# ska-sa/dc_sand

Measured on AMD Instinct MI355X. Metric: Gcoeff/s (complex weights) 64ant x 1024beam x 32768chan per GPU, higher is better.
Workload: dtype f32

## Files before the change

### dc_sand_amd/csrc/bf_beamform_i8_kernel.inc

```
template <int FORM, bool FULL, int NW = 4>
__global__ void __launch_bounds__(NW * 64) __attribute__((amdgpu_waves_per_eu(i8_waves_per_eu(FORM, FULL))))
#if BF_I8_WEIGHTED
bf_beamform_i8_w_kernel(const bf_bacc_args a, const bf_weights_args w)
#else
bf_beamform_i8_kernel(const bf_bacc_args a)
#endif
{
    constexpr bool WEIGHTED = BF_I8_WEIGHTED;
#if !BF_I8_WEIGHTED
    const bf_weights_args w{};
#endif
    static_assert(NW == 4 || ((NW == 8 || NW == 16) && FORM == kStaged), "8- and 16-wave workgroups exist for the staged form only");
    static_assert(!WEIGHTED || FORM == kStaged || FORM == kChain, "weights exist for the product's forms only");
    constexpr bool STAGED = FORM == kStaged, SPLIT = FORM == kSplit, CHAIN = FORM == kChain;
    extern __shared__ __attribute__((aligned(16))) char staged[];
    uint32_t bid = BACC_LOGICAL_ID(a);
    const uint32_t wave = __builtin_amdgcn_readfirstlane(threadIdx.x >> 6);
    const uint32_t lane = threadIdx.x & 63u;
    const uint32_t bg = bid % a.n_bgroups;
    bid /= a.n_bgroups;
    const uint32_t tg = bid % a.n_tgroups;
    const uint32_t c = bid / a.n_tgroups;
    const uint32_t nbt_log2 = SPLIT || CHAIN ? 0u : a.nbt_log2;
    const uint32_t nbt = 1u << nbt_log2, tpr = SPLIT ? 1u : (uint32_t)NW >> nbt_log2;
    const uint32_t bt = SPLIT ? 0u : wave & (nbt - 1u), slot = SPLIT ? 0u : wave >> nbt_log2;
    const uint32_t kc = SPLIT || CHAIN ? wave : 0u;
    const uint32_t lm = lane & 15u, lg = lane >> 4;
    const uint32_t bw = (bg * nbt + bt) * 16u;
    const uint32_t tt0 = tg * a.tiles_per_wg;
    const uint32_t tt1 = min(tt0 + a.tiles_per_wg, a.nT16);
    const uint32_t n_blocks = tt1 > tt0 + slot ? (tt1 - tt0 - slot + tpr - 1u) / tpr : 0u;
    const bool idle = bw >= a.B || n_blocks == 0u;
    if (!STAGED && !CHAIN && idle) return;
    const bool has_chunk = !(SPLIT || CHAIN) || 64u * kc < a.A;
    if (STAGED) {
        typedef __attribute__((address_space(3))) void lds_void;
        typedef const __attribute__((address_space(1))) void glb_void;
        const uint32_t bytes = (tt1 - tt0) * a.A * 32u;
        const char *src = reinterpret_cast<const char *>(a.ant) + ((uint64_t)c * a.nT16 + tt0) * a.A * 32u;
        for (uint32_t k = wave; k * 1024u < bytes; k += (uint32_t)NW)
            __builtin_amdgcn_global_load_lds((glb_void *)(src + min(k * 1024u + lane * 16u, bytes - 16u)), (lds_void *)(staged + k * 1024u),
                                             16, 0, 0);
    }

    const uint32_t fw = a.flags[0];
    const uint32_t cls = (fw >> 2) == a.epoch ? (fw & 3u) : DCS_CLASS_FAST_LOW;
    const float fChan = (float)c;
    const float D = a.k.fDenominator, y = a.k.fRcpDenominator;
    const float inv = 1.0f / kFixScale;
    float fac[4] = {inv, inv, inv, inv};
    if constexpr (WEIGHTED && STAGED) {
#pragma unroll
        for (int r = 0; r < 4; r++) fac[r] = w.gs[min(bw + (lane >> 4) + 4u * (uint32_t)r, a.B - 1u)] * inv;
    } else if constexpr (WEIGHTED && CHAIN) {
        fac[0] = w.gs[min(bw + (lane & 15u), a.B - 1u)] * inv;
    }

    const bool shared_w = STAGED && a.share_off != 0u && tpr > 1u && cls != DCS_CLASS_SLOW;
    intx4 wre[3], wim[3];
#pragma unroll
    for (int d = 0; d < 3; d++) wre[d] = wim[d] = intx4{0, 0, 0, 0};
    bool bad_re = false, bad_im = false;
    auto make_coefficients = [&]() {
        const uint32_t beam = bw + 4u * (lm & 3u) + (lm >> 2);
        const bool beam_live = beam < a.B;
        const float *tp = a.terms + 2u * (uint64_t)min(beam, a.B - 1u);
        const float *gp = WEIGHTED ? w.gn + min(beam, a.B - 1u) : nullptr;
        auto planes = [](const uint32_t (&g)[4], uint32_t (&out)[3]) {
            const uint32_t t0 = __builtin_amdgcn_perm(g[1], g[0], 0x05010400u), t1 = __builtin_amdgcn_perm(g[1], g[0], 0x07030602u);
            const uint32_t t2 = __builtin_amdgcn_perm(g[3], g[2], 0x05010400u), t3 = __builtin_amdgcn_perm(g[3], g[2], 0x07030602u);
            out[2] = __builtin_amdgcn_perm(t2, t0, 0x05040100u);
            out[1] = __builtin_amdgcn_perm(t2, t0, 0x07060302u);
            out[0] = __builtin_amdgcn_perm(t3, t1, 0x05040100u);
        };
        auto four = [&](auto gen, auto track, uint32_t q, const floatx2 (&k4)[4], const float (&g4)[4], uint32_t (&nr)[3],
                        uint32_t (&ni)[3]) {
            uint32_t gr[4], gi[4];
#pragma unroll
            for (uint32_t z = 0; z < 4; z++) {
                float re, im;
                gen(k4[z].x, k4[z].y, re, im);
                if constexpr (WEIGHTED) re = g4[z] * re, im = g4[z] * im;
                if (decltype(track)::value) {
                    bad_re |= !(fabsf(re) <= 2.0f);
                    bad_im |= !(fabsf(im) <= 2.0f);
                }
                gr[z] = fixed_word(re), gi[z] = fixed_word(im);
            }
            planes(gr, nr), planes(gi, ni);
            if (!FULL) {
                uint32_t mask = 0;
#pragma unroll
                for (uint32_t z = 0; z < 4; z++) mask |= 64u * kc + 4u * (4u * q + z) + lg < a.A ? 0xffu << (8u * z) : 0u;
#pragma unroll
                for (int d = 0; d < 3; d++) nr[d] &= mask, ni[d] &= mask;
            }
        };
        auto generate = [&](auto gen, auto unrolled) {
            floatx2 kp[16];
            float gw[16];
#pragma unroll
            for (uint32_t z = 0; z < 16; z++) {
                const uint32_t ant = 64u * kc + 4u * z + lg;
                if constexpr (WEIGHTED) {
                    if (decltype(unrolled)::value && z >= 4u) continue;
                    gw[z] = gp[(uint64_t)min(ant, a.A - 1u) * a.B];
                }
                kp[z] = *reinterpret_cast<const floatx2 *>(tp + 2u * (uint64_t)min(ant, a.A - 1u) * a.B);
            }
            if (decltype(unrolled)::value) {
#pragma unroll
                for (uint32_t q = 0; q < 4; q++) {
                    if constexpr (WEIGHTED) {
                        if (q < 3u) {
#pragma unroll
                            for (uint32_t z = 4u * q + 4u; z < 4u * q + 8u; z++) {
                                const uint32_t ant = 64u * kc + 4u * z + lg;
                                gw[z] = gp[(uint64_t)min(ant, a.A - 1u) * a.B];
                                kp[z] = *reinterpret_cast<const floatx2 *>(tp + 2u * (uint64_t)min(ant, a.A - 1u) * a.B);
                            }
                        }
                    }
                    if (shared_w && (q & (tpr - 1u)) != slot) continue;
                    const floatx2 k4[4] = {kp[4 * q], kp[4 * q + 1], kp[4 * q + 2], kp[4 * q + 3]};
                    float g4[4] = {};
                    if constexpr (WEIGHTED) g4[0] = gw[4 * q], g4[1] = gw[4 * q + 1], g4[2] = gw[4 * q + 2], g4[3] = gw[4 * q + 3];
                    uint32_t nr[3], ni[3];
                    four(gen, std::false_type{}, q, k4, g4, nr, ni);
                    if constexpr (CHAIN) {
                        uint32_t *cw = reinterpret_cast<uint32_t *>(staged) + (kc * 6u * 64u + lane) * 4u + q;
#pragma unroll
                        for (int d = 0; d < 3; d++) cw[(uint32_t)d * 256u] = beam_live ? nr[d] : 0u, cw[(3u + (uint32_t)d) * 256u] = beam_live ? ni[d] : 0u;
                    } else {
#pragma unroll
                        for (int d = 0; d < 3; d++) wre[d][q] = (int)nr[d], wim[d][q] = (int)ni[d];
                    }
                }
            } else {
#pragma unroll 1
                for (uint32_t q = 0; q < 4; q++) {
                    const floatx2 k4[4] = {kp[0], kp[1], kp[2], kp[3]};
                    float g4[4] = {};
                    if constexpr (WEIGHTED) {
#pragma unroll
                        for (uint32_t z = 0; z < 4; z++) g4[z] = gp[(uint64_t)min(64u * kc + 4u * (4u * q + z) + lg, a.A - 1u) * a.B];
                    }
                    uint32_t nr[3], ni[3];
                    four(gen, std::true_type{}, q, k4, g4, nr, ni);
                    if constexpr (CHAIN) {
                        uint32_t *cw = reinterpret_cast<uint32_t *>(staged) + (kc * 6u * 64u + lane) * 4u + q;
#pragma unroll
                        for (int d = 0; d < 3; d++) cw[(uint32_t)d * 256u] = beam_live ? nr[d] : 0u, cw[(3u + (uint32_t)d) * 256u] = beam_live ? ni[d] : 0u;
                    } else {
#pragma unroll
                        for (int d = 0; d < 3; d++) {
                            wre[d] = intx4{wre[d][1], wre[d][2], wre[d][3], (int)nr[d]};
                            wim[d] = intx4{wim[d][1], wim[d][2], wim[d][3], (int)ni[d]};
                        }
                    }
#pragma unroll
                    for (uint32_t z = 0; z < 12; z++) kp[z] = kp[z + 4];
                }
            }
            if (!CHAIN && !beam_live) {
#pragma unroll
                for (int d = 0; d < 3; d++) wre[d] = wim[d] = intx4{0, 0, 0, 0};
            }
        };
        if (cls == DCS_CLASS_SLOW) {
            generate([&](float kx, float ky, float &re, float &im) { coeff_slow(kx, ky, fChan, D, re, im); }, std::false_type{});
        } else {
            dispatch_fast(a.k.uDiv3Exact != 0u, cls == DCS_CLASS_FAST_LOW, [&](auto div3, auto lowdeg) {
                generate([&](float kx, float ky, float &re, float &im) {
                    coeff_fast<decltype(div3)::value, decltype(lowdeg)::value>(kx, ky, fChan, D, y, re, im);
                }, std::true_type{});
            });
        }
    };

    const char *ant8 = reinterpret_cast<const char *>(a.ant);
    const uint32_t blk_bytes = a.A * 32u;
    const uint32_t m = lm & 7u;
    const bool second = lm >= 8u;
    const uint32_t last = n_blocks - 1u;
    const uint32_t voff = lg * 32u + m * 4u;
    uint32_t cur[2][16];
    auto arrived = [&](uint32_t (&v)[16]) {
        asm volatile("" : "+v"(v[0]), "+v"(v[1]), "+v"(v[2]), "+v"(v[3]), "+v"(v[4]), "+v"(v[5]), "+v"(v[6]), "+v"(v[7]));
        asm volatile("" : "+v"(v[8]), "+v"(v[9]), "+v"(v[10]), "+v"(v[11]), "+v"(v[12]), "+v"(v[13]), "+v"(v[14]), "+v"(v[15]));
    };
    auto fetch = [&](uint32_t (&dst)[16], uint32_t blk, uint32_t kc) {
        const uint32_t blkA = min(blk, last), blkB = min(blk + 1u, last);
        if (STAGED) {
            const uint32_t at = ((second ? blkB : blkA) * tpr + slot) * blk_bytes + m * 4u;
#pragma unroll
            for (uint32_t p = 0; p < 16; p++)
                dst[p] = *reinterpret_cast<const uint32_t *>(staged + at + (FULL ? lg + 4u * p : min(lg + 4u * p, a.A - 1u)) * 32u);
            return;
        }
        const char *base = ant8 + ((uint64_t)c * a.nT16 + tt0 + blkA * tpr + slot) * blk_bytes;
        const uint32_t hop = second ? (blkB - blkA) * tpr * blk_bytes : 0u;
        if (FULL) {
            const char *b2 = base + 2048u * kc;
            const uint32_t vo = hop + voff;
#pragma unroll
            for (uint32_t p = 0; p < 16; p++) dst[p] = *reinterpret_cast<const uint32_t *>(b2 + vo + 128u * p);
        } else {
#pragma unroll
            for (uint32_t p = 0; p < 16; p++)
                dst[p] = *reinterpret_cast<const uint32_t *>(base + (hop + min(64u * kc + lg + 4u * p, a.A - 1u) * 32u + m * 4u));
        }
    };
    auto transpose = [&](const uint32_t (&v)[16], intx4 (&x)[4]) {
#pragma unroll
        for (int q = 0; q < 4; q++) {
            const uint32_t t0 = __builtin_amdgcn_perm(v[4 * q + 1], v[4 * q], 0x05010400u);
            const uint32_t t1 = __builtin_amdgcn_perm(v[4 * q + 1], v[4 * q], 0x07030602u);
            const uint32_t t2 = __builtin_amdgcn_perm(v[4 * q + 3], v[4 * q + 2], 0x05010400u);
            const uint32_t t3 = __builtin_amdgcn_perm(v[4 * q + 3], v[4 * q + 2], 0x07030602u);
            x[0][q] = (int)__builtin_amdgcn_perm(t2, t0, 0x05040100u);
            x[1][q] = (int)__builtin_amdgcn_perm(t2, t0, 0x07060302u);
            x[2][q] = (int)__builtin_amdgcn_perm(t3, t1, 0x05040100u);
            x[3][q] = (int)__builtin_amdgcn_perm(t3, t1, 0x07060302u);
        }
    };
    const intx4 zero = {0, 0, 0, 0};
    auto contract = [&](const intx4 (&x)[4], floatx4 (&f)[4]) {
#pragma unroll
        for (int v = 0; v < 4; v++) {
            const intx4 s3 = __builtin_amdgcn_mfma_i32_16x16x64_i8((v & 1) ? wim[2] : wre[2], x[v], zero, 0, 0, 0);
            const intx4 s2 = __builtin_amdgcn_mfma_i32_16x16x64_i8((v & 1) ? wim[1] : wre[1], x[v], zero, 0, 0, 0);
            const intx4 s1 = __builtin_amdgcn_mfma_i32_16x16x64_i8((v & 1) ? wim[0] : wre[0], x[v], zero, 0, 0, 0);
#pragma unroll
            for (int r = 0; r < 4; r++) f[v][r] = fmaf((float)s1[r], 65536.0f, (float)(s2[r] * 256 + s3[r]));
        }
    };
    uint32_t nan_re = 0, nan_im = 0;
    const float fNaN = __builtin_nanf("");
    auto poison = [&](int r, floatx4 &o) {
        if ((nan_re >> (4u * lg + (uint32_t)r)) & 1u) o[0] = fNaN, o[2] = fNaN;
        if ((nan_im >> (4u * lg + (uint32_t)r)) & 1u) o[1] = fNaN, o[3] = fNaN;
    };
    const uint32_t bb = bw + lg;
    const uint32_t out_blk = a.B * 128u;
    char *out8 = reinterpret_cast<char *>(a.beams);
    auto out_of = [&](uint32_t blk, int r) {
        const uint32_t blkA = min(blk, last), blkB = min(blk + 1u, last);
        char *base = out8 + ((uint64_t)c * a.nT16 + tt0 + blkA * tpr + slot) * out_blk;
        return reinterpret_cast<floatx4 *>(base + ((second ? (blkB - blkA) * tpr * out_blk : 0u) + bb * 128u + m * 16u + 512u * r));
    };
    auto store = [&](floatx4 *dst, const floatx4 o) {
#ifdef DCS_PROBES
        if (a.plain_stores) {
            *dst = o;
            return;
        }
#endif
        __builtin_nontemporal_store(o, dst);
    };
    auto finish = [&](auto whole, uint32_t blk, const floatx4 (&f)[4]) {
#pragma unroll
        for (int r = 0; r < 4; r++) {
            const float sc = WEIGHTED ? fac[r] : inv;
            floatx4 o = {f[0][r] * sc, f[1][r] * sc, f[2][r] * sc, f[3][r] * sc};
            if (nan_re | nan_im) poison(r, o);
            if (decltype(whole)::value || bb + 4u * r < a.B) {
                floatx4 *dst = out_of(blk, r);
#ifdef DCS_PROBES
                if (a.probe == 4u) {
                    const uint32_t blkA = min(blk, last), blkB = min(blk + 1u, last);
                    dst = reinterpret_cast<floatx4 *>(out8 + ((uint64_t)c * a.nT16 + tt0 + blkA * tpr + slot) * out_blk +
                                                      ((r >= 2 ? (blkB - blkA) * tpr * out_blk : 0u) + bw * 128u + (r & 1) * 1024u + lane * 16u));
                }
#endif
                store(dst, o);
            }
        }
    };
    floatx4 *part = reinterpret_cast<floatx4 *>(staged);
    const uint32_t n_chunks = (a.A + 63u) / 64u;
    auto park = [&](int h, const floatx4 (&f)[4]) {
#pragma unroll
        for (int r = 0; r < 4; r++) {
            floatx4 o = {f[0][r], f[1][r], f[2][r], f[3][r]};
            if (nan_re | nan_im) poison(r, o);
            part[((h * 4 + r) * 4 + kc) * 64u + lane] = o;
        }
    };
    auto gather = [&](auto whole, int h, uint32_t blk) {
        floatx4 o = part[((h * 4 + wave) * 4 + 0) * 64u + lane];
        for (uint32_t k = 1; k < n_chunks; k++) o = o + part[((h * 4 + wave) * 4 + k) * 64u + lane];
        o = o * inv;
        if (decltype(whole)::value || bb + 4u * wave < a.B) store(out_of(blk, (int)wave), o);
    };
    auto run = [&](auto whole) {
#ifdef DCS_PROBES
        if (!SPLIT && (a.probe == 1u || a.probe == 3u || a.probe == 4u)) {
            floatx4 f[4];
#pragma unroll
            for (int v = 0; v < 4; v++) f[v] = floatx4{(float)wre[0][0], (float)wre[1][1], (float)wim[0][2], (float)wim[2][3]};
            for (uint32_t blk = 0; blk < n_blocks; blk += 2) finish(whole, blk, f);
            return;
        }
        if (FORM == kDirect && a.probe == 2u) {
            for (uint32_t blk = 0; blk < n_blocks; blk += 4) {
                arrived(cur[0]);
                arrived(cur[1]);
#pragma unroll
                for (int h = 0; h < 2; h++) {
                    floatx4 f[4];
#pragma unroll
                    for (int v = 0; v < 4; v++)
                        f[v] = floatx4{(float)cur[h][4 * v], (float)cur[h][4 * v + 1], (float)cur[h][4 * v + 2], (float)cur[h][4 * v + 3]};
                    finish(whole, blk + 2u * h, f);
                }
                __builtin_amdgcn_sched_barrier(0);
                fetch(cur[0], blk + 4u, kc);
                fetch(cur[1], blk + 6u, kc);
            }
            return;
        }
#endif
        if (STAGED) {
            for (uint32_t blk = 0; blk < n_blocks; blk += 2) {
                intx4 x[4];
                floatx4 f[4];
                fetch(cur[0], blk, 0u);
                transpose(cur[0], x);
                contract(x, f);
                finish(whole, blk, f);
            }
        } else {
            for (uint32_t blk = 0; blk < n_blocks; blk += 4) {
                if (has_chunk) {
                    arrived(cur[0]);
                    arrived(cur[1]);
#pragma unroll
                    for (int h = 0; h < 2; h++) {
                        intx4 x[4];
                        floatx4 f[4];
                        transpose(cur[h], x);
                        contract(x, f);
                        if (SPLIT)
                            park(h, f);
                        else
                            finish(whole, blk + 2u * h, f);
                    }
                }
                if (SPLIT) {
                    __syncthreads();
                    gather(whole, 0, blk);
                    gather(whole, 1, blk + 2u);
                    __syncthreads();
                }
                __builtin_amdgcn_sched_barrier(0);
                if (has_chunk) {
                    fetch(cur[0], blk + 4u, kc);
                    fetch(cur[1], blk + 6u, kc);
                }
            }
        }
    };
    if (!STAGED && !CHAIN && has_chunk) fetch(cur[0], 0, kc);
    if (CHAIN && !idle) fetch(cur[0], 0, 0u);
    __builtin_amdgcn_sched_barrier(0);
#ifdef DCS_PROBES
    if (a.probe == 3u || a.probe == 4u) {
#pragma unroll
        for (int d = 0; d < 3; d++) wre[d] = wim[d] = intx4{(int)lane, d, 2, 1};
    } else
#endif
    if ((shared_w || CHAIN ? bw < a.B : !idle) && has_chunk) make_coefficients();
    if (cls == DCS_CLASS_SLOW) {
        const uint64_t br = __builtin_amdgcn_ballot_w64(bad_re), bi = __builtin_amdgcn_ballot_w64(bad_im);
        nan_re = (uint32_t)((br | (br >> 16) | (br >> 32) | (br >> 48)) & 0xffffu);
        nan_im = (uint32_t)((bi | (bi >> 16) | (bi >> 32) | (bi >> 48)) & 0xffffu);
    }
    if constexpr (STAGED) {
        uint32_t *wx = reinterpret_cast<uint32_t *>(staged + a.share_off) + bt * (4u * 6u * 64u) + lane;
        if (shared_w && bw < a.B) {
#pragma unroll
            for (uint32_t q = 0; q < 4; q++)
                if ((q & (tpr - 1u)) == slot) {
#pragma unroll
                    for (int d = 0; d < 3; d++) wx[(q * 6u + d) * 64u] = (uint32_t)wre[d][q], wx[(q * 6u + 3u + d) * 64u] = (uint32_t)wim[d][q];
                }
        }
        __syncthreads();
        if (idle) return;
        if (shared_w) {
#pragma unroll
            for (uint32_t q = 0; q < 4; q++)
                if ((q & (tpr - 1u)) != slot) {
#pragma unroll
                    for (int d = 0; d < 3; d++) wre[d][q] = (int)wx[(q * 6u + d) * 64u], wim[d][q] = (int)wx[(q * 6u + 3u + d) * 64u];
                }
        }
    } else if constexpr (CHAIN) {
        intx4 *coef = reinterpret_cast<intx4 *>(staged);
        uint32_t *nanw = reinterpret_cast<uint32_t *>(staged + 4u * 6u * 64u * 16u);
        if (lane == 0u) nanw[2u * wave] = has_chunk ? nan_re : 0u, nanw[2u * wave + 1u] = has_chunk ? nan_im : 0u;
        float *facw = reinterpret_cast<float *>(nanw + 8);
        if constexpr (WEIGHTED) {
            if (wave == 0u && lane < 16u) facw[lane] = fac[0];
        }
        __syncthreads();
        if (idle) return;
        nan_re = nanw[0] | nanw[2] | nanw[4] | nanw[6];
        nan_im = nanw[1] | nanw[3] | nanw[5] | nanw[7];
        const uint32_t n_chunks = (a.A + 63u) / 64u;
        auto run_chain = [&](auto whole) {
            const uint32_t n_steps = ((n_blocks + 1u) >> 1) * n_chunks;
            intx4 acc[4][3];
            uint32_t s = 0, chunk = 0, blk = 0;
            uint32_t f_s = 1u, f_chunk = 1u % n_chunks, f_blk = 2u * (1u / n_chunks);
            auto step = [&](uint32_t (&now)[16], uint32_t (&ahead)[16]) {
                arrived(now);
                if (f_s < n_steps) fetch(ahead, f_blk, f_chunk);
                f_s++;
                if (++f_chunk == n_chunks) f_chunk = 0u, f_blk += 2u;
                intx4 x[4];
                transpose(now, x);
                if (chunk == 0u) {
#pragma unroll
                    for (int v = 0; v < 4; v++)
#pragma unroll
                        for (int d = 0; d < 3; d++) acc[v][d] = zero;
                }
#pragma unroll
                for (int half = 0; half < 2; half++) {
#pragma unroll
                    for (int d = 0; d < 3; d++) {
                        const intx4 w = coef[(chunk * 6u + 3u * (uint32_t)half + (uint32_t)d) * 64u + lane];
#pragma unroll
                        for (int v = half; v < 4; v += 2) acc[v][d] = __builtin_amdgcn_mfma_i32_16x16x64_i8(w, x[v], acc[v][d], 0, 0, 0);
                    }
                }
                if (chunk + 1u == n_chunks) {
                    float sc_next = WEIGHTED ? facw[lg] : inv;
#pragma unroll
                    for (int r = 0; r < 4; r++) {
                        const float sc = sc_next;
                        if constexpr (WEIGHTED) {
                            if (r < 3) sc_next = facw[4u * (uint32_t)r + 4u + lg];
                        }
                        floatx4 o;
#pragma unroll
                        for (int v = 0; v < 4; v++) o[v] = fmaf((float)acc[v][0][r], 65536.0f, (float)(acc[v][1][r] * 256 + acc[v][2][r])) * sc;
                        if (nan_re | nan_im) poison(r, o);
                        if (decltype(whole)::value || bb + 4u * (uint32_t)r < a.B) store(out_of(blk, r), o);
                        __builtin_amdgcn_sched_barrier(0);
                    }
                    chunk = 0u, blk += 2u;
                } else {
                    chunk++;
                }
                s++;
            };
            while (s < n_steps) {
                step(cur[0], cur[1]);
                if (s < n_steps) step(cur[1], cur[0]);
            }
        };
        if (bw + 16u <= a.B)
            run_chain(std::true_type{});
        else
            run_chain(std::false_type{});
        return;
    } else if (has_chunk) {
        fetch(cur[1], 2, kc);
    }
    if (bw + 16u <= a.B)
        run(std::true_type{});
    else
        run(std::false_type{});
}
```

### dc_sand_amd/csrc/bf_beamform_mfma.hip

```cpp

#include "bf_kernels.h"

#include <hip/hip_runtime.h>

#include <type_traits>

#include "bf_device.h"

namespace {

__device__ __forceinline__ uint32_t xcd_grouped(uint32_t w, uint32_t total, uint32_t G) { return bf_xcd_grouped(w, total, G); }
#ifdef DCS_PROBES
__device__ __forceinline__ uint32_t probe_order(uint32_t order, uint32_t w, uint32_t total, uint32_t G, uint32_t n_sharers)
{
    if (order == 1u) return w;
    if (order >= 16u && order < 24u) return (w + (order - 16u)) % total;
    if (order == 2u) {
        const uint32_t per = total >> 3, rem = total & 7u, x = w & 7u, q = w >> 3;
        return x * per + min(x, rem) + q;
    }
    return xcd_grouped(w, total, order == 3u ? n_sharers : G);
}
#define BACC_LOGICAL_ID(a) probe_order((a).order, blockIdx.x, gridDim.x, (a).xcd_group, (a).n_bgroups)
#else
#define BACC_LOGICAL_ID(a) xcd_grouped(blockIdx.x, gridDim.x, (a).xcd_group)
#endif

constexpr uint32_t kKC = 64;

template <int NBT>
__global__ void __launch_bounds__(kBlock) bf_beamform_acc_kernel(const bf_bacc_args a)
{
    constexpr int TPR = 4 / NBT;
    constexpr uint32_t WS = 16u * NBT + (NBT > 1 ? 16u : 0u);
    constexpr uint32_t NJ = kKC / 4u;
    extern __shared__ __attribute__((aligned(16))) float lds[];
    const uint32_t A_pad = (a.A + 3u) & ~3u;

    uint32_t bid = BACC_LOGICAL_ID(a);
    const uint32_t bg = bid % a.n_bgroups;
    bid /= a.n_bgroups;
    const uint32_t tg = bid % a.n_tgroups;
    const uint32_t c = bid / a.n_tgroups;
    const uint32_t b0 = bg * 16u * NBT;
    const uint32_t tt0 = tg * a.tiles_per_wg;
    const uint32_t tt1 = min(tt0 + a.tiles_per_wg, a.nT16);

    const uint32_t wave = threadIdx.x >> 6, lane = threadIdx.x & 63u;
    const uint32_t bt = wave % NBT, slot = wave / NBT;
    const uint32_t lm = lane & 15u, lg = lane >> 4;

    const uint32_t fw = a.flags[0];
    const uint32_t cls = (fw >> 2) == a.epoch ? (fw & 3u) : DCS_CLASS_FAST_LOW;
    const float fChan = (float)c;
    const float D = a.k.fDenominator, y = a.k.fRcpDenominator;
    auto with_generator = [&](auto &&body) {
        if (cls == DCS_CLASS_SLOW) {
            body([&](float kx, float ky, float &re, float &im) { coeff_slow(kx, ky, fChan, D, re, im); });
        } else {
            dispatch_fast(a.k.uDiv3Exact != 0u, cls == DCS_CLASS_FAST_LOW, [&](auto div3, auto lowdeg) {
                body([&](float kx, float ky, float &re, float &im) {
                    coeff_fast<decltype(div3)::value, decltype(lowdeg)::value>(kx, ky, fChan, D, y, re, im);
                });
            });
        }
    };

    {
        float *Wre = lds, *Wim = lds + (size_t)A_pad * WS;
        const uint32_t nb = 16u * NBT;
        with_generator([&](auto gen) {
            constexpr uint32_t kBatch = 8;
            for (uint32_t i0 = threadIdx.x; i0 < A_pad * nb; i0 += kBlock * kBatch) {
                floatx2 kp[kBatch];
#pragma unroll
                for (uint32_t q = 0; q < kBatch; q++) {
                    const uint32_t i = min(i0 + q * kBlock, A_pad * nb - 1u), ant = i / nb, b = b0 + (i - ant * nb);
                    kp[q] = *reinterpret_cast<const floatx2 *>(a.terms + 2u * ((uint64_t)min(ant, a.A - 1u) * a.B + min(b, a.B - 1u)));
                }
#pragma unroll 1
                for (uint32_t q = 0; q < kBatch; q++) {
                    const uint32_t i = i0 + q * kBlock, ant = i / nb, bl = i - ant * nb;
                    floatx2 t = kp[0];
#pragma unroll
                    for (uint32_t z = 1; z < kBatch; z++) t = (z == q) ? kp[z] : t;
                    float re, im;
                    gen(t.x, t.y, re, im);
                    if (i < A_pad * nb) {
                        const bool live = ant < a.A && b0 + bl < a.B;
                        Wre[ant * WS + bl] = live ? re : 0.0f;
                        Wim[ant * WS + bl] = live ? im : 0.0f;
                    }
                }
            }
        });
        __syncthreads();
    }
    const uint32_t n_chunks = (a.A + kKC - 1u) / kKC;
    const uint32_t n_blocks = tt1 > tt0 + slot ? (tt1 - tt0 - slot + TPR - 1u) / TPR : 0u;
    const uint32_t n_stages = n_blocks * n_chunks;
    const uint16_t *ant16 = reinterpret_cast<const uint16_t *>(a.ant);
    uint32_t cur[NJ], nxt[NJ];
    auto fetch = [&](uint32_t s, uint32_t (&dst)[NJ]) {
        const uint32_t tt = tt0 + (s / n_chunks) * TPR + slot, a0 = (s % n_chunks) * kKC;
        const uint16_t *p0 = ant16 + ((uint64_t)c * a.nT16 + tt) * a.A * 16u + lm;
        if (a0 + kKC <= a.A) {
            const uint16_t *p = p0 + (size_t)(a0 + lg) * 16u;
#pragma unroll
            for (uint32_t j = 0; j < NJ; j++) dst[j] = p[(size_t)j * 64u];
        } else {
#pragma unroll
            for (uint32_t j = 0; j < NJ; j++) dst[j] = p0[(size_t)min(a0 + lg + 4u * j, a.A - 1u) * 16u];
        }
    };
    floatx4 acc_re = {0.0f, 0.0f, 0.0f, 0.0f}, acc_im = {0.0f, 0.0f, 0.0f, 0.0f};
    if (n_stages) fetch(0, cur);
    for (uint32_t s = 0; s < n_stages; s++) {
        const uint32_t blk = s / n_chunks, chunk = s - blk * n_chunks, a0 = chunk * kKC;
        if (s + 1 < n_stages) fetch(s + 1, nxt);
        const float *wr = lds + (size_t)(a0 + lg) * WS + bt * 16u + lm;
        const float *wi = wr + (size_t)A_pad * WS;
        if (a0 + kKC <= a.A) {
#pragma unroll
            for (uint32_t j = 0; j < NJ; j++) {
                acc_re = __builtin_amdgcn_mfma_f32_16x16x4f32(wr[(size_t)j * 4u * WS], (float)(int8_t)(cur[j] & 0xffu), acc_re, 0, 0, 0);
                acc_im = __builtin_amdgcn_mfma_f32_16x16x4f32(wi[(size_t)j * 4u * WS], (float)(int8_t)(cur[j] >> 8), acc_im, 0, 0, 0);
            }
        } else {
            const uint32_t nj = (a.A - a0 + 3u) >> 2;
            for (uint32_t j = 0; j < nj; j++) {
                uint32_t v = cur[0];
#pragma unroll
                for (uint32_t z = 1; z < NJ; z++) v = (z == j) ? cur[z] : v;
                v &= 0u - (uint32_t)(a0 + lg + 4u * j < a.A);
                acc_re = __builtin_amdgcn_mfma_f32_16x16x4f32(wr[(size_t)j * 4u * WS], (float)(int8_t)(v & 0xffu), acc_re, 0, 0, 0);
                acc_im = __builtin_amdgcn_mfma_f32_16x16x4f32(wi[(size_t)j * 4u * WS], (float)(int8_t)(v >> 8), acc_im, 0, 0, 0);
            }
        }
        if (chunk + 1 == n_chunks) {
            floatx2 *dst = reinterpret_cast<floatx2 *>(a.beams) + ((uint64_t)c * a.nT16 + tt0 + blk * TPR + slot) * a.B * 16u + lm;
            const uint32_t bb = b0 + bt * 16u + lg * 4u;
#pragma unroll
            for (int r = 0; r < 4; r++)
                if (bb + r < a.B) dst[(uint64_t)(bb + r) * 16u] = floatx2{acc_re[r], acc_im[r]};
            acc_re = floatx4{0.0f, 0.0f, 0.0f, 0.0f};
            acc_im = floatx4{0.0f, 0.0f, 0.0f, 0.0f};
        }
#pragma unroll
        for (uint32_t j = 0; j < NJ; j++) cur[j] = nxt[j];
    }
}


typedef int intx4 __attribute__((ext_vector_type(4)));
constexpr float kFixScale = 8355711.0f;

__device__ __forceinline__ uint32_t fixed_word(float w)
{
    const float f = __builtin_amdgcn_fmed3f(w * kFixScale, -kFixScale, kFixScale);
    return ((uint32_t)(int)rintf(f) + 0x808080u) ^ 0x808080u;
}

enum { kStaged = 0, kDirect = 1, kSplit = 2, kChain = 3 };
constexpr int kChainWaves = 4;

constexpr int i8_waves_per_eu(int form, bool full)
{
    return form == kSplit ? (full ? 3 : 2) : (form == kChain ? kChainWaves : (full || form == kStaged ? 4 : 3));
}

#define BF_I8_WEIGHTED 0
#include "bf_beamform_i8_kernel.inc"
#undef BF_I8_WEIGHTED
#define BF_I8_WEIGHTED 1
#include "bf_beamform_i8_kernel.inc"
#undef BF_I8_WEIGHTED

}

static size_t bacc_lds_bytes(int nbt, uint32_t A)
{
    const uint32_t A_pad = (A + 3u) & ~3u;
    const uint32_t ws = 16u * (uint32_t)nbt + (nbt > 1 ? 16u : 0u);
    return (size_t)A_pad * ws * 2u * sizeof(float);
}

hipError_t bf_warm_module_mfma()
{
    hipFuncAttributes attr;
    return hipFuncGetAttributes(&attr, reinterpret_cast<const void *>(&bf_beamform_i8_kernel<kStaged, true>));
}

namespace {
hipError_t launch_beamform_acc(const bf_bacc_args &a_in, const bf_weights_args *w, hipStream_t stream)
{
    bf_bacc_args a = a_in;
    if (a.A == 0 || a.B == 0 || a.C == 0 || a.nT16 == 0) return hipSuccess;
    if (a.A > 256u) return hipErrorInvalidValue;
    const bool chain = a.fp32_chain != 0u;
    if (w && chain) return hipErrorInvalidValue;
    const bool wide = !chain && a.A > 64u;
    const bool split = wide && BACC_KNOB(a, unstaged) != 0u;
    const bool staged_form = !chain && a.A <= 64u && !BACC_KNOB(a, unstaged);
    int nbt = wide ? 1 : (a.B > 32u ? 4 : (a.B > 16u ? 2 : 1));
#ifdef DCS_PROBES
    if (staged_form && (a.nbt_force == 1u || a.nbt_force == 2u || a.nbt_force == 4u || a.nbt_force == 8u)) nbt = (int)a.nbt_force;
#endif
    uint32_t nw = nbt == 8 ? 8u : 4u;
#ifdef DCS_PROBES
    if (staged_form && (a.nw_force == 8u || a.nw_force == 16u) && a.nw_force >= (uint32_t)nbt) nw = a.nw_force;
#endif
    while (chain && nbt > 1 && bacc_lds_bytes(nbt, a.A) > 26u * 1024u) nbt >>= 1;
    const size_t lds = chain ? bacc_lds_bytes(nbt, a.A) : 0u;
    a.nbt_log2 = nbt == 8 ? 3u : (nbt == 4 ? 2u : (nbt == 2 ? 1u : 0u));
    a.n_bgroups = (a.B + 16u * (uint32_t)nbt - 1u) / (16u * (uint32_t)nbt);
    const uint32_t tpr = split ? 1u : nw / (uint32_t)nbt;
    const uint32_t blocks_cap = staged_form && nbt == 4 && a.n_bgroups == 1u ? 8u : 16u;
    const uint32_t max_rounds = BACC_KNOB(a, max_rounds) ? BACC_KNOB(a, max_rounds) : (chain ? 16u : (staged_form || wide ? blocks_cap / tpr : 32u));
    uint32_t tiles = (a.nT16 + tpr - 1u) / tpr * tpr;
    if (tiles > max_rounds * tpr) {
        const uint32_t parts = (a.nT16 + max_rounds * tpr - 1u) / (max_rounds * tpr);
        tiles = ((a.nT16 + parts - 1u) / parts + tpr - 1u) / tpr * tpr;
    }
    const uint64_t enough = chain ? 4096u : 5120u / nw;
    while (tiles > tpr && (uint64_t)a.C * a.n_bgroups * ((a.nT16 + tiles - 1u) / tiles) < enough) tiles = ((tiles / tpr + 1u) / 2u) * tpr;
    a.tiles_per_wg = tiles;
    a.n_tgroups = (a.nT16 + tiles - 1u) / tiles;
    a.xcd_group = wide ? a.n_bgroups : (!chain && a.n_bgroups >= 16u ? a.n_bgroups : 1u);
    const uint64_t blocks = (uint64_t)a.C * a.n_bgroups * a.n_tgroups;
    if (blocks > 0x7fffffffull) return hipErrorInvalidValue;
    const dim3 grid((uint32_t)blocks), block(64u * nw);
    if (w) {
        if (nw != 4u || (!staged_form && (!wide || split))) return hipErrorInvalidValue;
        if (staged_form) {
            size_t stage_bytes = ((size_t)a.tiles_per_wg * a.A * 32u + 1023u) / 1024u * 1024u;
            if (tpr > 1u && !BACC_KNOB(a, no_share)) {
                a.share_off = (uint32_t)stage_bytes;
                stage_bytes += (size_t)nbt * 4u * 6u * 64u * sizeof(uint32_t);
            }
            if (a.A == 64u)
                hipLaunchKernelGGL((bf_beamform_i8_w_kernel<kStaged, true>), grid, block, stage_bytes, stream, a, *w);
            else
                hipLaunchKernelGGL((bf_beamform_i8_w_kernel<kStaged, false>), grid, block, stage_bytes, stream, a, *w);
        } else {
            const size_t coef_bytes = 4u * 6u * 64u * 16u + 8u * sizeof(uint32_t) + 16u * sizeof(float);
            if (a.A % 64u == 0u)
                hipLaunchKernelGGL((bf_beamform_i8_w_kernel<kChain, true>), grid, block, coef_bytes, stream, a, *w);
            else
                hipLaunchKernelGGL((bf_beamform_i8_w_kernel<kChain, false>), grid, block, coef_bytes, stream, a, *w);
        }
        return hipGetLastError();
    }
    if (chain) {
        if (nbt == 4)
            hipLaunchKernelGGL(bf_beamform_acc_kernel<4>, grid, block, lds, stream, a);
        else if (nbt == 2)
            hipLaunchKernelGGL(bf_beamform_acc_kernel<2>, grid, block, lds, stream, a);
        else
            hipLaunchKernelGGL(bf_beamform_acc_kernel<1>, grid, block, lds, stream, a);
    } else if (staged_form) {
        size_t stage_bytes = ((size_t)a.tiles_per_wg * a.A * 32u + 1023u) / 1024u * 1024u;
        if (tpr > 1u && !BACC_KNOB(a, no_share)) {
            a.share_off = (uint32_t)stage_bytes;
            stage_bytes += (size_t)nbt * 4u * 6u * 64u * sizeof(uint32_t);
        }
#ifdef DCS_PROBES
        if (a.wg_per_cu >= 1u && a.wg_per_cu <= 5u && stage_bytes < 160u * 1024u / a.wg_per_cu)
            stage_bytes = (160u * 1024u / a.wg_per_cu) & ~1023u;
#endif
#ifdef DCS_PROBES
        if (nw == 8u) {
            if (a.A == 64u)
                hipLaunchKernelGGL((bf_beamform_i8_kernel<kStaged, true, 8>), grid, block, stage_bytes, stream, a);
            else
                hipLaunchKernelGGL((bf_beamform_i8_kernel<kStaged, false, 8>), grid, block, stage_bytes, stream, a);
        } else if (nw == 16u) {
            if (a.A == 64u)
                hipLaunchKernelGGL((bf_beamform_i8_kernel<kStaged, true, 16>), grid, block, stage_bytes, stream, a);
            else
                hipLaunchKernelGGL((bf_beamform_i8_kernel<kStaged, false, 16>), grid, block, stage_bytes, stream, a);
        } else
#endif
        if (a.A == 64u)
            hipLaunchKernelGGL((bf_beamform_i8_kernel<kStaged, true>), grid, block, stage_bytes, stream, a);
        else
            hipLaunchKernelGGL((bf_beamform_i8_kernel<kStaged, false>), grid, block, stage_bytes, stream, a);
#ifdef DCS_PROBES
    } else if (a.A <= 64u) {
        if (a.A == 64u)
            hipLaunchKernelGGL((bf_beamform_i8_kernel<kDirect, true>), grid, block, 0, stream, a);
        else
            hipLaunchKernelGGL((bf_beamform_i8_kernel<kDirect, false>), grid, block, 0, stream, a);
#endif
#ifdef DCS_PROBES
    } else if (split) {
        const size_t part_bytes = 2u * 4u * 4u * 64u * 16u;
        if (a.A % 64u == 0u)
            hipLaunchKernelGGL((bf_beamform_i8_kernel<kSplit, true>), grid, block, part_bytes, stream, a);
        else
            hipLaunchKernelGGL((bf_beamform_i8_kernel<kSplit, false>), grid, block, part_bytes, stream, a);
#endif
    } else {
        const size_t coef_bytes = 4u * 6u * 64u * 16u + 8u * sizeof(uint32_t);
        if (a.A % 64u == 0u)
            hipLaunchKernelGGL((bf_beamform_i8_kernel<kChain, true>), grid, block, coef_bytes, stream, a);
        else
            hipLaunchKernelGGL((bf_beamform_i8_kernel<kChain, false>), grid, block, coef_bytes, stream, a);
    }
    return hipGetLastError();
}
}

hipError_t bf_launch_beamform_acc(const bf_bacc_args &a, hipStream_t stream) { return launch_beamform_acc(a, nullptr, stream); }

hipError_t bf_launch_beamform_acc_weighted(const bf_bacc_args &a, const bf_weights_args &w, hipStream_t stream)
{
    return launch_beamform_acc(a, &w, stream);
}
```

Baseline: 927.7.

## Process two beam tiles per workgroup in the chain kernel to reuse antenna data

Measured after the change: 928.9 (median of 4 runs). About the same (+0.1%).

```diff
diff --git a/dc_sand_amd/csrc/bf_beamform_i8_kernel.inc b/dc_sand_amd/csrc/bf_beamform_i8_kernel.inc
--- a/dc_sand_amd/csrc/bf_beamform_i8_kernel.inc
+++ b/dc_sand_amd/csrc/bf_beamform_i8_kernel.inc
@@ -1,5 +1,5 @@
-template <int FORM, bool FULL, int NW = 4>
-__global__ void __launch_bounds__(NW * 64) __attribute__((amdgpu_waves_per_eu(i8_waves_per_eu(FORM, FULL))))
+template <int FORM, bool FULL, int NW = 4, int CT = 1>
+__global__ void __launch_bounds__(NW * 64) __attribute__((amdgpu_waves_per_eu(i8_waves_per_eu(FORM, FULL, CT))))
 #if BF_I8_WEIGHTED
 bf_beamform_i8_w_kernel(const bf_bacc_args a, const bf_weights_args w)
 #else
@@ -12,6 +12,7 @@
 #endif
     static_assert(NW == 4 || ((NW == 8 || NW == 16) && FORM == kStaged), "8- and 16-wave workgroups exist for the staged form only");
     static_assert(!WEIGHTED || FORM == kStaged || FORM == kChain, "weights exist for the product's forms only");
+    static_assert(CT == 1 || ((CT == 2 || CT == 4) && FORM == kChain), "several beam tiles per wave exist for kChain only");
     constexpr bool STAGED = FORM == kStaged, SPLIT = FORM == kSplit, CHAIN = FORM == kChain;
     extern __shared__ __attribute__((aligned(16))) char staged[];
     uint32_t bid = BACC_LOGICAL_ID(a);
@@ -26,7 +27,7 @@
     const uint32_t bt = SPLIT ? 0u : wave & (nbt - 1u), slot = SPLIT ? 0u : wave >> nbt_log2;
     const uint32_t kc = SPLIT || CHAIN ? wave : 0u;
     const uint32_t lm = lane & 15u, lg = lane >> 4;
-    const uint32_t bw = (bg * nbt + bt) * 16u;
+    const uint32_t bw = CHAIN ? bg * 16u * (uint32_t)CT : (bg * nbt + bt) * 16u;
     const uint32_t tt0 = tg * a.tiles_per_wg;
     const uint32_t tt1 = min(tt0 + a.tiles_per_wg, a.nT16);
     const uint32_t n_blocks = tt1 > tt0 + slot ? (tt1 - tt0 - slot + tpr - 1u) / tpr : 0u;
@@ -53,7 +54,7 @@
 #pragma unroll
         for (int r = 0; r < 4; r++) fac[r] = w.gs[min(bw + (lane >> 4) + 4u * (uint32_t)r, a.B - 1u)] * inv;
     } else if constexpr (WEIGHTED && CHAIN) {
-        fac[0] = w.gs[min(bw + (lane & 15u), a.B - 1u)] * inv;
+        fac[0] = w.gs[min(bw + (lane & (16u * CT - 1u)), a.B - 1u)] * inv;
     }
 
     const bool shared_w = STAGED && a.share_off != 0u && tpr > 1u && cls != DCS_CLASS_SLOW;
@@ -61,8 +62,11 @@
 #pragma unroll
     for (int d = 0; d < 3; d++) wre[d] = wim[d] = intx4{0, 0, 0, 0};
     bool bad_re = false, bad_im = false;
+    uint32_t tm = 0;
+    const uint32_t tile_ops = CHAIN ? (a.A + 63u) / 64u * 6u * 64u : 0u;
+    constexpr uint32_t kChainHead = CT == 1 ? 0u : 96u * CT;
     auto make_coefficients = [&]() {
-        const uint32_t beam = bw + 4u * (lm & 3u) + (lm >> 2);
+        const uint32_t beam = (CHAIN ? bw + 16u * tm : bw) + 4u * (lm & 3u) + (lm >> 2);
         const bool beam_live = beam < a.B;
         const float *tp = a.terms + 2u * (uint64_t)min(beam, a.B - 1u);
         const float *gp = WEIGHTED ? w.gn + min(beam, a.B - 1u) : nullptr;
@@ -128,7 +132,7 @@
                     uint32_t nr[3], ni[3];
                     four(gen, std::false_type{}, q, k4, g4, nr, ni);
                     if constexpr (CHAIN) {
-                        uint32_t *cw = reinterpret_cast<uint32_t *>(staged) + (kc * 6u * 64u + lane) * 4u + q;
+                        uint32_t *cw = reinterpret_cast<uint32_t *>(staged + kChainHead) + (tm * tile_ops + kc * 6u * 64u + lane) * 4u + q;
 #pragma unroll
                         for (int d = 0; d < 3; d++) cw[(uint32_t)d * 256u] = beam_live ? nr[d] : 0u, cw[(3u + (uint32_t)d) * 256u] = beam_live ? ni[d] : 0u;
                     } else {
@@ -148,7 +152,7 @@
                     uint32_t nr[3], ni[3];
                     four(gen, std::true_type{}, q, k4, g4, nr, ni);
                     if constexpr (CHAIN) {
-                        uint32_t *cw = reinterpret_cast<uint32_t *>(staged) + (kc * 6u * 64u + lane) * 4u + q;
+                        uint32_t *cw = reinterpret_cast<uint32_t *>(staged + kChainHead) + (tm * tile_ops + kc * 6u * 64u + lane) * 4u + q;
 #pragma unroll
                         for (int d = 0; d < 3; d++) cw[(uint32_t)d * 256u] = beam_live ? nr[d] : 0u, cw[(3u + (uint32_t)d) * 256u] = beam_live ? ni[d] : 0u;
                     } else {
@@ -370,8 +374,8 @@
         for (int d = 0; d < 3; d++) wre[d] = wim[d] = intx4{(int)lane, d, 2, 1};
     } else
 #endif
-    if ((shared_w || CHAIN ? bw < a.B : !idle) && has_chunk) make_coefficients();
-    if (cls == DCS_CLASS_SLOW) {
+    if (!CHAIN && (shared_w ? bw < a.B : !idle) && has_chunk) make_coefficients();
+    if (!CHAIN && cls == DCS_CLASS_SLOW) {
         const uint64_t br = __builtin_amdgcn_ballot_w64(bad_re), bi = __builtin_amdgcn_ballot_w64(bad_im);
         nan_re = (uint32_t)((br | (br >> 16) | (br >> 32) | (br >> 48)) & 0xffffu);
         nan_im = (uint32_t)((bi | (bi >> 16) | (bi >> 32) | (bi >> 48)) & 0xffffu);
@@ -397,21 +401,47 @@
                 }
         }
     } else if constexpr (CHAIN) {
-        intx4 *coef = reinterpret_cast<intx4 *>(staged);
-        uint32_t *nanw = reinterpret_cast<uint32_t *>(staged + 4u * 6u * 64u * 16u);
-        if (lane == 0u) nanw[2u * wave] = has_chunk ? nan_re : 0u, nanw[2u * wave + 1u] = has_chunk ? nan_im : 0u;
-        float *facw = reinterpret_cast<float *>(nanw + 8);
+        uint32_t *nanw = reinterpret_cast<uint32_t *>(staged + (CT == 1 ? 4u * 6u * 64u * 16u : 0u));
+        float *facw = reinterpret_cast<float *>(nanw + 8 * CT);
+        intx4 *coef = reinterpret_cast<intx4 *>(staged + kChainHead);
+        auto make_tile = [&]() {
+            bad_re = bad_im = false;
+            nan_re = nan_im = 0u;
+#ifdef DCS_PROBES
+            if (a.probe != 3u && a.probe != 4u)
+#endif
+            if (bw + 16u * tm < a.B && has_chunk) make_coefficients();
+            if (cls == DCS_CLASS_SLOW) {
+                const uint64_t br = __builtin_amdgcn_ballot_w64(bad_re), bi = __builtin_amdgcn_ballot_w64(bad_im);
+                nan_re = (uint32_t)((br | (br >> 16) | (br >> 32) | (br >> 48)) & 0xffffu);
+                nan_im = (uint32_t)((bi | (bi >> 16) | (bi >> 32) | (bi >> 48)) & 0xffffu);
+            }
+            if (lane == 0u) nanw[8u * tm + 2u * wave] = has_chunk ? nan_re : 0u, nanw[8u * tm + 2u * wave + 1u] = has_chunk ? nan_im : 0u;
+        };
+        if constexpr (CT == 1) {
+            make_tile();
+        } else {
+#pragma unroll 1
+            for (tm = 0; tm < (uint32_t)CT; tm++) make_tile();
+        }
         if constexpr (WEIGHTED) {
-            if (wave == 0u && lane < 16u) facw[lane] = fac[0];
+            if (wave == 0u && lane < 16u * CT) facw[lane] = fac[0];
         }
         __syncthreads();
         if (idle) return;
-        nan_re = nanw[0] | nanw[2] | nanw[4] | nanw[6];
-        nan_im = nanw[1] | nanw[3] | nanw[5] | nanw[7];
+        uint32_t nan_t[CT][2];
+#pragma unroll
+        for (int t = 0; t < CT; t++) {
+            const uint32_t *nw = nanw + 8 * t;
+            nan_t[t][0] = nw[0] | nw[2] | nw[4] | nw[6];
+            nan_t[t][1] = nw[1] | nw[3] | nw[5] | nw[7];
+        }
+        nan_re = nan_t[0][0], nan_im = nan_t[0][1];
         const uint32_t n_chunks = (a.A + 63u) / 64u;
+        auto tile_live = [&](int t) { return t == 0 || bw + 16u * (uint32_t)t < a.B; };
         auto run_chain = [&](auto whole) {
             const uint32_t n_steps = ((n_blocks + 1u) >> 1) * n_chunks;
-            intx4 acc[4][3];
+            intx4 acc[CT][4][3];
             uint32_t s = 0, chunk = 0, blk = 0;
             uint32_t f_s = 1u, f_chunk = 1u % n_chunks, f_blk = 2u * (1u / n_chunks);
             auto step = [&](uint32_t (&now)[16], uint32_t (&ahead)[16]) {
@@ -423,33 +453,46 @@
                 transpose(now, x);
                 if (chunk == 0u) {
 #pragma unroll
-                    for (int v = 0; v < 4; v++)
-#pragma unroll
-                        for (int d = 0; d < 3; d++) acc[v][d] = zero;
-                }
-#pragma unroll
-                for (int half = 0; half < 2; half++) {
-#pragma unroll
-                    for (int d = 0; d < 3; d++) {
-                        const intx4 w = coef[(chunk * 6u + 3u * (uint32_t)half + (uint32_t)d) * 64u + lane];
-#pragma unroll
-                        for (int v = half; v < 4; v += 2) acc[v][d] = __builtin_amdgcn_mfma_i32_16x16x64_i8(w, x[v], acc[v][d], 0, 0, 0);
+                    for (int t = 0; t < CT; t++)
+#pragma unroll
+                        for (int v = 0; v < 4; v++)
+#pragma unroll
+                            for (int d = 0; d < 3; d++) acc[t][v][d] = zero;
+                }
+#pragma unroll
+                for (int t = 0; t < CT; t++) {
+                    if (!tile_live(t)) continue;
+                    const intx4 *ct = coef + (uint32_t)t * tile_ops + chunk * 6u * 64u + lane;
+#pragma unroll
+                    for (int half = 0; half < 2; half++) {
+#pragma unroll
+                        for (int d = 0; d < 3; d++) {
+                            const intx4 w = ct[(3u * (uint32_t)half + (uint32_t)d) * 64u];
+#pragma unroll
+                            for (int v = half; v < 4; v += 2) acc[t][v][d] = __builtin_amdgcn_mfma_i32_16x16x64_i8(w, x[v], acc[t][v][d], 0, 0, 0);
+                        }
                     }
                 }
                 if (chunk + 1u == n_chunks) {
-                    float sc_next = WEIGHTED ? facw[lg] : inv;
-#pragma unroll
-                    for (int r = 0; r < 4; r++) {
-                        const float sc = sc_next;
-                        if constexpr (WEIGHTED) {
-                            if (r < 3) sc_next = facw[4u * (uint32_t)r + 4u + lg];
+#pragma unroll
+                    for (int t = 0; t < CT; t++) {
+                        if (!tile_live(t)) continue;
+                        if constexpr (CT > 1) nan_re = nan_t[t][0], nan_im = nan_t[t][1];
+                        const float *ft = facw + 16 * t;
+                        float sc_next = WEIGHTED ? ft[lg] : inv;
+#pragma unroll
+                        for (int r = 0; r < 4; r++) {
+                            const float sc = sc_next;
+                            if constexpr (WEIGHTED) {
+                                if (r < 3) sc_next = ft[4u * (uint32_t)r + 4u + lg];
+                            }
+                            floatx4 o;
+#pragma unroll
+                            for (int v = 0; v < 4; v++) o[v] = fmaf((float)acc[t][v][0][r], 65536.0f, (float)(acc[t][v][1][r] * 256 + acc[t][v][2][r])) * sc;
+                            if (nan_re | nan_im) poison(r, o);
+                            if (decltype(whole)::value || bb + 16u * (uint32_t)t + 4u * (uint32_t)r < a.B) store(out_of(blk, r) + 128u * (uint32_t)t, o);
+                            __builtin_amdgcn_sched_barrier(0);
                         }
-                        floatx4 o;
-#pragma unroll
-                        for (int v = 0; v < 4; v++) o[v] = fmaf((float)acc[v][0][r], 65536.0f, (float)(acc[v][1][r] * 256 + acc[v][2][r])) * sc;
-                        if (nan_re | nan_im) poison(r, o);
-                        if (decltype(whole)::value || bb + 4u * (uint32_t)r < a.B) store(out_of(blk, r), o);
-                        __builtin_amdgcn_sched_barrier(0);
                     }
                     chunk = 0u, blk += 2u;
                 } else {
@@ -462,7 +505,7 @@
                 if (s < n_steps) step(cur[1], cur[0]);
             }
         };
-        if (bw + 16u <= a.B)
+        if (bw + 16u * CT <= a.B)
             run_chain(std::true_type{});
         else
             run_chain(std::false_type{});
diff --git a/dc_sand_amd/csrc/bf_beamform_mfma.hip b/dc_sand_amd/csrc/bf_beamform_mfma.hip
--- a/dc_sand_amd/csrc/bf_beamform_mfma.hip
+++ b/dc_sand_amd/csrc/bf_beamform_mfma.hip
@@ -162,11 +162,12 @@
 }
 
 enum { kStaged = 0, kDirect = 1, kSplit = 2, kChain = 3 };
-constexpr int kChainWaves = 4;
-
-constexpr int i8_waves_per_eu(int form, bool full)
-{
-    return form == kSplit ? (full ? 3 : 2) : (form == kChain ? kChainWaves : (full || form == kStaged ? 4 : 3));
+constexpr int kChainWaves[3] = {4, 2, 1};
+constexpr size_t kChainLds = 50u * 1024u;
+
+constexpr int i8_waves_per_eu(int form, bool full, int ct)
+{
+    return form == kSplit ? (full ? 3 : 2) : (form == kChain ? kChainWaves[ct >> 1] : (full || form == kStaged ? 4 : 3));
 }
 
 #define BF_I8_WEIGHTED 0
@@ -185,10 +186,58 @@
     return (size_t)A_pad * ws * 2u * sizeof(float);
 }
 
+static size_t chain_lds_bytes(int ct, uint32_t A)
+{
+    if (ct == 1) return 4u * 6u * 1024u + 8u * sizeof(uint32_t) + 16u * sizeof(float);
+    return (size_t)ct * (8u * sizeof(uint32_t) + 16u * sizeof(float) + (A + 63u) / 64u * 6u * 1024u);
+}
+
+namespace {
+template <int CT, bool FULL>
+hipError_t allow_chain_lds()
+{
+    const int bytes = (int)chain_lds_bytes(CT, 256u);
+    hipError_t e = hipFuncSetAttribute(reinterpret_cast<const void *>(&bf_beamform_i8_kernel<kChain, FULL, 4, CT>),
+                                       hipFuncAttributeMaxDynamicSharedMemorySize, bytes);
+    if (e == hipSuccess)
+        e = hipFuncSetAttribute(reinterpret_cast<const void *>(&bf_beamform_i8_w_kernel<kChain, FULL, 4, CT>),
+                                hipFuncAttributeMaxDynamicSharedMemorySize, bytes);
+    return e;
+}
+
+template <int CT, bool FULL>
+void launch_chain(const bf_bacc_args &a, const bf_weights_args *w, dim3 grid, dim3 block, size_t lds, hipStream_t stream)
+{
+    if constexpr (CT > 1) {
+        if (w) {
+            hipLaunchKernelGGL((bf_beamform_i8_w_kernel<kChain, FULL, 4, CT>), grid, block, lds, stream, a, *w);
+            return;
+        }
+    }
+    hipLaunchKernelGGL((bf_beamform_i8_kernel<kChain, FULL, 4, CT>), grid, block, lds, stream, a);
+}
+
+template <int CT>
+void launch_chain_tiles(const bf_bacc_args &a, const bf_weights_args *w, dim3 grid, dim3 block, size_t lds, hipStream_t stream)
+{
+    if (a.A % 64u == 0u)
+        launch_chain<CT, true>(a, w, grid, block, lds, stream);
+    else
+        launch_chain<CT, false>(a, w, grid, block, lds, stream);
+}
+}
+
 hipError_t bf_warm_module_mfma()
 {
     hipFuncAttributes attr;
-    return hipFuncGetAttributes(&attr, reinterpret_cast<const void *>(&bf_beamform_i8_kernel<kStaged, true>));
+    hipError_t e = hipFuncGetAttributes(&attr, reinterpret_cast<const void *>(&bf_beamform_i8_kernel<kStaged, true>));
+    if (e == hipSuccess) e = allow_chain_lds<2, true>();
+    if (e == hipSuccess) e = allow_chain_lds<2, false>();
+#ifdef DCS_PROBES
+    if (e == hipSuccess) e = allow_chain_lds<4, true>();
+    if (e == hipSuccess) e = allow_chain_lds<4, false>();
+#endif
+    return e;
 }
 
 namespace {
@@ -212,8 +261,16 @@
 #endif
     while (chain && nbt > 1 && bacc_lds_bytes(nbt, a.A) > 26u * 1024u) nbt >>= 1;
     const size_t lds = chain ? bacc_lds_bytes(nbt, a.A) : 0u;
+    int ct = 1;
+    if (wide && !split) {
+        ct = (a.B > 16u || w) && chain_lds_bytes(2, a.A) <= kChainLds ? 2 : 1;
+#ifdef DCS_PROBES
+        if (a.nbt_force == 1u || a.nbt_force == 2u || a.nbt_force == 4u) ct = (int)a.nbt_force;
+        if (w && ct == 1) ct = 2;
+#endif
+    }
     a.nbt_log2 = nbt == 8 ? 3u : (nbt == 4 ? 2u : (nbt == 2 ? 1u : 0u));
-    a.n_bgroups = (a.B + 16u * (uint32_t)nbt - 1u) / (16u * (uint32_t)nbt);
+    a.n_bgroups = (a.B + 16u * (uint32_t)(nbt * ct) - 1u) / (16u * (uint32_t)(nbt * ct));
     const uint32_t tpr = split ? 1u : nw / (uint32_t)nbt;
     const uint32_t blocks_cap = staged_form && nbt == 4 && a.n_bgroups == 1u ? 8u : 16u;
     const uint32_t max_rounds = BACC_KNOB(a, max_rounds) ? BACC_KNOB(a, max_rounds) : (chain ? 16u : (staged_form || wide ? blocks_cap / tpr : 32u));
@@ -243,11 +300,16 @@
             else
                 hipLaunchKernelGGL((bf_beamform_i8_w_kernel<kStaged, false>), grid, block, stage_bytes, stream, a, *w);
         } else {
-            const size_t coef_bytes = 4u * 6u * 64u * 16u + 8u * sizeof(uint32_t) + 16u * sizeof(float);
-            if (a.A % 64u == 0u)
-                hipLaunchKernelGGL((bf_beamform_i8_w_kernel<kChain, true>), grid, block, coef_bytes, stream, a, *w);
-            else
-                hipLaunchKernelGGL((bf_beamform_i8_w_kernel<kChain, false>), grid, block, coef_bytes, stream, a, *w);
+            const size_t coef_bytes = chain_lds_bytes(ct, a.A);
+#ifdef DCS_PROBES
+            if (ct == 4)
+                launch_chain_tiles<4>(a, w, grid, block, coef_bytes, stream);
+            else
+#endif
+            if (ct == 2)
+                launch_chain_tiles<2>(a, w, grid, block, coef_bytes, stream);
+            else
+                return hipErrorInvalidValue;
         }
         return hipGetLastError();
     }
@@ -301,11 +363,16 @@
             hipLaunchKernelGGL((bf_beamform_i8_kernel<kSplit, false>), grid, block, part_bytes, stream, a);
 #endif
     } else {
-        const size_t coef_bytes = 4u * 6u * 64u * 16u + 8u * sizeof(uint32_t);
-        if (a.A % 64u == 0u)
-            hipLaunchKernelGGL((bf_beamform_i8_kernel<kChain, true>), grid, block, coef_bytes, stream, a);
-        else
-            hipLaunchKernelGGL((bf_beamform_i8_kernel<kChain, false>), grid, block, coef_bytes, stream, a);
+        const size_t coef_bytes = chain_lds_bytes(ct, a.A);
+#ifdef DCS_PROBES
+        if (ct == 4)
+            launch_chain_tiles<4>(a, nullptr, grid, block, coef_bytes, stream);
+        else
+#endif
+        if (ct == 2)
+            launch_chain_tiles<2>(a, nullptr, grid, block, coef_bytes, stream);
+        else
+            launch_chain_tiles<1>(a, nullptr, grid, block, coef_bytes, stream);
     }
     return hipGetLastError();
 }
```
